# vinhisreal/YOLO-LitePi

Hardware: AMD Instinct MI355X
Metric: images/sec end-to-end (det+NMS+clf) 640x640 batch64 (higher is better)
Workload: dtype f16; 1 GPU; configs[2]: full det+NMS+ROI+ShuffleNetV2 pipeline, fp16, batch=64/GPU, 640x640, inputs resident in HBM; classifier=ShuffleNetV2 x1.0, 91 classes, seeded random weights, 64x64 ROIs, min_area=50, max_det=300, steps_in_flight=3, distinct_input_batches=4, global_batch=64, boxes_pre_area_filter_rank0=413

## Files before the change

yolo-litepi_amd/csrc/cls_net.h:

```cpp
#pragma once
#include "cls_fused.h"
#include "common.h"

namespace lp {

struct FusedS2W {
  const float* dw1;
  const float* dw1b;
  const u32x4_t* pwb1;
  const float* pwb1b;
  const u32x4_t* pw1;
  const float* pw1b;
  const float* dw2;
  const float* dw2b;
  const u32x4_t* pw2;
  const float* pw2b;
};

struct ClsFrontArgs {
  const uint8_t* rgb;
  const int* m_dyn;
  void* out;
  const u32x4_t* stem_w;
  const float* stem_b;
  FusedS2W s20;
  FusedBlockW s2[3];
  FusedS2W s30;
};

struct ClsBackArgs {
  const void* in;
  const int* m_dyn;
  FusedBlockW s3[7];
  FusedS2W s40;
  FusedBlockW s4[3];
  const u32x4_t* w5;
  const float* b5;
  const u32x4_t* wfc;
  const float* bfc;
  float* probs;
  int* ids;
  float* logits;
  lp_det* dets;
  const int* roi_img;
  const int* roi_slot;
  int max_det, nc, nc_p, logits_pitch;
};

void launch_cls_front(const ClsFrontArgs& a, int max_items, hipStream_t st);
void launch_cls_back(const ClsBackArgs& a, int max_items, hipStream_t st);
void pack_cls_stem(const std::vector<float>& w_oihw, const std::vector<float>& bias, std::vector<uint16_t>& frags, std::vector<float>& bias_cases);

}
```

yolo-litepi_amd/csrc/cls_net.hip:

```cpp
#include "cls_net.h"

namespace lp {

typedef _Float16 half_t;
typedef _Float16 half8 __attribute__((ext_vector_type(8)));
typedef _Float16 half4 __attribute__((ext_vector_type(4)));
typedef _Float16 half2v __attribute__((ext_vector_type(2)));
typedef float floatx4 __attribute__((ext_vector_type(4)));
typedef uint32_t u32x4 __attribute__((ext_vector_type(4)));

#define CN_THREADS 512
#define CN_WAVES 8

#define BF2 58
#define BFP2 64
#define BF3 116
#define BFP3 128
#define BF4 232
#define BFP4 240

template <int SMAX>
__device__ __forceinline__ void wload(u32x4 (&af)[SMAX], const u32x4_t* __restrict__ w, int t, int S, int lane) {
#pragma unroll
  for (int s = 0; s < SMAX; ++s) {
    af[s] = u32x4{0u, 0u, 0u, 0u};
    if (s < S) af[s] = w[((size_t)t * S + s) * 64 + lane];
  }
}

template <int SMAX, int PT>
__device__ __forceinline__ void gemm_acc(const u32x4 (&af)[SMAX], int S, int s0, const char* bsrc, int brow, int Kp, int p0, int lane,
                                         floatx4 (&acc)[PT]) {
  const int g = lane >> 4, col = lane & 15;
#pragma unroll
  for (int s = 0; s < SMAX; ++s) {
    if (s < S) {
      const half8 a = __builtin_bit_cast(half8, af[s]);
      const int kg = 4 * (s0 + s) + g;
#pragma unroll
      for (int p = 0; p < PT; ++p) {
        u32x4 v = u32x4{0u, 0u, 0u, 0u};
        if (kg * 8 < Kp) v = *reinterpret_cast<const u32x4*>(bsrc + (p0 + p * 16 + col) * brow + kg * 16);
        acc[p] = __builtin_amdgcn_mfma_f32_16x16x32_f16(a, __builtin_bit_cast(half8, v), acc[p], 0, 0, 0);
      }
    }
  }
}

template <int PT> __device__ __forceinline__ void zero_acc(floatx4 (&acc)[PT]) {
#pragma unroll
  for (int p = 0; p < PT; ++p) acc[p] = floatx4{0.f, 0.f, 0.f, 0.f};
}

template <int PT>
__device__ __forceinline__ void store_relu(char* dst, int drow, int p0, int t, const float* __restrict__ bias, const floatx4 (&acc)[PT],
                                           int lane) {
  const int g = lane >> 4, col = lane & 15;
  const int ch0 = t * 16 + 4 * g;
  const floatx4 b = *reinterpret_cast<const floatx4*>(bias + ch0);
#pragma unroll
  for (int p = 0; p < PT; ++p) {
    half4 q;
#pragma unroll
    for (int i = 0; i < 4; ++i) q[i] = (half_t)fmaxf(acc[p][i] + b[i], 0.f);
    *reinterpret_cast<half4*>(dst + (p0 + p * 16 + col) * drow + ch0 * 2) = q;
  }
}

template <int C, int WIN, int WOUT, int STRIDE>
__device__ __forceinline__ void dwconv(const char* in, int irow, char* out, int orow, const float* __restrict__ w,
                                       const float* __restrict__ b, int nroi, int tid) {
  constexpr int CG = C / 8;
  const int items = nroi * WOUT * WOUT * CG;
  for (int i = tid; i < items; i += CN_THREADS) {
    const int cg = i % CG, px = i / CG;
    const int r = px / (WOUT * WOUT), pp = px - r * (WOUT * WOUT);
    const int oy = pp / WOUT, ox = pp - oy * WOUT;
    float acc[8];
    {
      const floatx4 b0 = *reinterpret_cast<const floatx4*>(b + cg * 8), b1 = *reinterpret_cast<const floatx4*>(b + cg * 8 + 4);
#pragma unroll
      for (int j = 0; j < 4; ++j) { acc[j] = b0[j]; acc[4 + j] = b1[j]; }
    }
#pragma unroll 1
    for (int ky = 0; ky < 3; ++ky) {
      const int iy = oy * STRIDE - 1 + ky;
      if (iy < 0 || iy >= WIN) continue;
      const char* rowp = in + ((r * WIN + iy) * WIN) * irow + cg * 16;
      const float* wrow = w + (ky * 3) * C + cg * 8;
#pragma unroll
      for (int kx = 0; kx < 3; ++kx) {
        const int ix = ox * STRIDE - 1 + kx;
        const bool ok = ix >= 0 && ix < WIN;
        u32x4 raw = u32x4{0u, 0u, 0u, 0u};
        if (ok) raw = *reinterpret_cast<const u32x4*>(rowp + ix * irow);
        const half8 v = __builtin_bit_cast(half8, raw);
        const floatx4 w0 = *reinterpret_cast<const floatx4*>(wrow + kx * C);
        const floatx4 w1 = *reinterpret_cast<const floatx4*>(wrow + kx * C + 4);
#pragma unroll
        for (int j = 0; j < 4; ++j) {
          acc[j] = fmaf((float)v[j], w0[j], acc[j]);
          acc[4 + j] = fmaf((float)v[4 + j], w1[j], acc[4 + j]);
        }
      }
    }
    half8 o;
#pragma unroll
    for (int j = 0; j < 8; ++j) o[j] = (half_t)acc[j];
    *reinterpret_cast<half8*>(out + px * orow + cg * 16) = o;
  }
}

__device__ __forceinline__ int shuffle_phys(int l, int bf, int bfp) { return l < bf ? l : bfp + (l - bf); }

template <int BFP, int NB>
__device__ __forceinline__ void stage_biases(float* BI, const FusedBlockW* blk, int tid) {
  constexpr int Q = BFP / 4;
  for (int i = tid; i < NB * 2 * Q; i += CN_THREADS) {
    const int b = i / (2 * Q), rem = i - b * 2 * Q, which = rem / Q, j = rem - which * Q;
    const float* src = which ? blk[b].b2 : blk[b].b1;
    *reinterpret_cast<floatx4*>(BI + (size_t)(b * 2 + which) * BFP + 4 * j) = *reinterpret_cast<const floatx4*>(src + 4 * j);
  }
}

template <int C>
__device__ __forceinline__ void stage_dw(float* dst, const float* __restrict__ w, const float* __restrict__ b, int tid) {
  constexpr int Q = 10 * C / 4;
  for (int i = tid; i < Q; i += CN_THREADS)
    *reinterpret_cast<floatx4*>(dst + 4 * i) = i < 9 * C / 4 ? *reinterpret_cast<const floatx4*>(w + 4 * i) : *reinterpret_cast<const floatx4*>(b + 4 * (i - 9 * C / 4));
}

template <int BF, int BFP, int W, int PT, int ROUNDS, bool PREF = true>
__device__ __forceinline__ void s1_block(char* X, int xrow, char* T1, char* T2, int trow, const FusedBlockW& bw, const u32x4_t* w1n, int nroi,
                                         int p0, int tile0, int tstride, u32x4 (&f1)[ROUNDS][BFP / 32 + ((BFP % 32) ? 1 : 0)], int tid, float* DW, const float* BI) {
  constexpr int TT = BFP / 16, S = BFP / 32 + ((BFP % 32) ? 1 : 0);
  const int lane = tid & 63;
  const int g = lane >> 4, col = lane & 15;
  constexpr int NDW4 = 10 * BFP / 4, DWPT = (NDW4 + CN_THREADS - 1) / CN_THREADS;
  floatx4 dwreg[DWPT];
#pragma unroll
  for (int k = 0; k < DWPT; ++k) {
    int idx = tid + k * CN_THREADS;
    idx = idx < NDW4 ? idx : NDW4 - 1;
    dwreg[k] = idx < 9 * BFP / 4 ? *reinterpret_cast<const floatx4*>(bw.dw + 4 * idx) : *reinterpret_cast<const floatx4*>(bw.dwb + 4 * (idx - 9 * BFP / 4));
  }
  u32x4 f2[ROUNDS][S];
  floatx4 acc[ROUNDS][PT];
  int tc[ROUNDS];
  bool live[ROUNDS];
#pragma unroll
  for (int r = 0; r < ROUNDS; ++r) {
    const int t = tile0 + r * tstride;
    live[r] = t < TT;
    tc[r] = live[r] ? t : TT - 1;
  }
  if (PREF) {
#pragma unroll
    for (int r = 0; r < ROUNDS; ++r) wload<S>(f2[r], bw.w2, tc[r], S, lane);
  } else {
#pragma unroll
    for (int r = 0; r < ROUNDS; ++r) wload<S>(f1[r], bw.w1, tc[r], S, lane);
  }
#pragma unroll
  for (int r = 0; r < ROUNDS; ++r) {
    zero_acc<PT>(acc[r]);
    gemm_acc<S, PT>(f1[r], S, 0, X + BFP * 2, xrow, BFP, p0, lane, acc[r]);
    if (live[r]) store_relu<PT>(T1, trow, p0, tc[r], BI, acc[r], lane);
  }
  asm volatile("" ::: "memory");
  if (PREF) {
    if (w1n) {
#pragma unroll
      for (int r = 0; r < ROUNDS; ++r) wload<S>(f1[r], w1n, tc[r], S, lane);
    }
  } else {
#pragma unroll
    for (int r = 0; r < ROUNDS; ++r) wload<S>(f2[r], bw.w2, tc[r], S, lane);
  }
#pragma unroll
  for (int k = 0; k < DWPT; ++k) {
    const int idx = tid + k * CN_THREADS;
    if (idx < NDW4) *reinterpret_cast<floatx4*>(DW + 4 * idx) = dwreg[k];
  }
  __syncthreads();
  dwconv<BFP, W, W, 1>(T1, trow, T2, trow, DW, DW + 9 * BFP, nroi, tid);
  __syncthreads();
  half4 x1v[ROUNDS][PT];
#pragma unroll
  for (int r = 0; r < ROUNDS; ++r) {
    zero_acc<PT>(acc[r]);
    gemm_acc<S, PT>(f2[r], S, 0, T2, trow, BFP, p0, lane, acc[r]);
#pragma unroll
    for (int p = 0; p < PT; ++p) x1v[r][p] = *reinterpret_cast<const half4*>(X + (p0 + p * 16 + col) * xrow + (tc[r] * 16 + 4 * g) * 2);
  }
  __syncthreads();
#pragma unroll
  for (int r = 0; r < ROUNDS; ++r) {
    if (live[r]) {
      const int ch0 = tc[r] * 16 + 4 * g;
      const floatx4 bias = *reinterpret_cast<const floatx4*>(BI + BFP + ch0);
#pragma unroll
      for (int p = 0; p < PT; ++p) {
#pragma unroll
        for (int i = 0; i < 4; ++i) {
          const int c = ch0 + i;
          if (c < BF) {
            half2v pr;
            pr[0] = x1v[r][p][i];
            pr[1] = (half_t)fmaxf(acc[r][p][i] + bias[i], 0.f);
            *reinterpret_cast<half2v*>(X + (p0 + p * 16 + col) * xrow + shuffle_phys(2 * c, BF, BFP) * 2) = pr;
          }
        }
      }
    }
  }
  __syncthreads();
}

#define CF_IN 16
#define CF_RA 12352
#define CF_POOL (CF_RA + 49152)
#define CF_X2 (CF_POOL + 16384)
#define CF_LDS (CF_X2 + 17408)
#define CF_DW (10 * 64 * 4)
#define CF_BI (3 * 2 * 64 * 4)
#define CF_S2 ((10 * 24 + 10 * 64 + 10 * 128 + 10 * 128) * 4)
#define CF_POOLROW 64
#define CF_T1ROW 144
#define CF_X2ROW 272
#define CF_X3ROW 528

__global__ __launch_bounds__(CN_THREADS) void cls_front_kernel(const ClsFrontArgs a) {
  extern __shared__ __attribute__((aligned(16))) char smem[];
  const int tid0 = threadIdx.x, lane0 = tid0 & 63;
  const int R = *a.m_dyn;
  if ((int)blockIdx.x >= R) return;
  char* IN = smem + CF_IN;
  char* RA = smem + CF_RA;
  char* POOL = smem + CF_POOL;
  char* X2 = smem + CF_X2;
  char* T2 = smem;
  for (int i = tid0; i < 64 * CF_X2ROW / 16; i += CN_THREADS) *reinterpret_cast<u32x4*>(X2 + i * 16) = u32x4{0u, 0u, 0u, 0u};
  if (tid0 < 2) *reinterpret_cast<u32x4*>(smem + (tid0 ? CF_IN + 12288 : 0)) = u32x4{0u, 0u, 0u, 0u};
  stage_biases<BFP2, 3>(reinterpret_cast<float*>(smem + CF_LDS + CF_DW), a.s2, tid0);
  float* S2P = reinterpret_cast<float*>(smem + CF_LDS + CF_DW + CF_BI);
  stage_dw<24>(S2P, a.s20.dw1, a.s20.dw1b, tid0);
  stage_dw<64>(S2P + 240, a.s20.dw2, a.s20.dw2b, tid0);
  stage_dw<128>(S2P + 240 + 640, a.s30.dw1, a.s30.dw1b, tid0);
  stage_dw<128>(S2P + 240 + 640 + 1280, a.s30.dw2, a.s30.dw2b, tid0);
  const half8 sa0 = __builtin_bit_cast(half8, a.stem_w[lane0]), sa1 = __builtin_bit_cast(half8, a.stem_w[64 + lane0]);

  for (int r = blockIdx.x; r < R; r += gridDim.x) {
    int tid = tid0, lane = lane0;
    asm volatile("" : "+v"(tid), "+v"(lane));
    const int wave = __builtin_amdgcn_readfirstlane(tid >> 6);
    const int g = lane >> 4, col = lane & 15;
    {
      const u32x4* src = reinterpret_cast<const u32x4*>(a.rgb + (size_t)r * 12288);
      for (int i = tid; i < 768; i += CN_THREADS) *reinterpret_cast<u32x4*>(IN + i * 16) = src[i];
    }
    u32x4 fpw1[1];
    wload<1>(fpw1, a.s20.pw1, wave & 3, 1, lane);
    __syncthreads();

    for (int pt = wave * 8; pt < wave * 8 + 8; ++pt) {
      const int oy = pt >> 1, ox = (pt & 1) * 16 + col;
      const int b0 = 6 * ox - 3;
      uint32_t w0 = 0u, w1 = 0u;
      if (g < 3) {
        const int iy = 2 * oy - 1 + g;
        const int sh = b0 & 3, al = b0 - sh;
        const char* rowp = IN + (iy < 0 ? 0 : iy) * 192 + al;
        const uint32_t d0 = *reinterpret_cast<const uint32_t*>(rowp), d1 = *reinterpret_cast<const uint32_t*>(rowp + 4),
                       d2 = *reinterpret_cast<const uint32_t*>(rowp + 8);
        w0 = __builtin_amdgcn_alignbyte(d1, d0, sh);
        w1 = __builtin_amdgcn_alignbyte(d2, d1, sh);
        if (ox == 0) w0 &= 0xFF000000u;
        if (iy < 0) { w0 = 0u; w1 = 0u; }
      } else {
#pragma unroll
        for (int ky = 0; ky < 3; ++ky) {
          const int iy = 2 * oy - 1 + ky;
          const uint32_t v = iy < 0 ? 0u : (uint32_t) * reinterpret_cast<const uint8_t*>(IN + iy * 192 + b0 + 8);
          w0 |= v << (8 * ky);
        }
      }
      typedef uint32_t u32x4l __attribute__((ext_vector_type(4)));
      u32x4l hb;
      hb[0] = __builtin_amdgcn_perm(0x64646464u, w0, 0x04010400u);
      hb[1] = __builtin_amdgcn_perm(0x64646464u, w0, 0x04030402u);
      hb[2] = __builtin_amdgcn_perm(0x64646464u, w1, 0x04010400u);
      hb[3] = __builtin_amdgcn_perm(0x64646464u, w1, 0x04030402u);
      half8 bf = __builtin_bit_cast(half8, hb);
#pragma unroll
      for (int j = 0; j < 8; ++j) bf[j] = bf[j] - (half_t)1024.f;
      floatx4 c0 = floatx4{0.f, 0.f, 0.f, 0.f}, c1 = floatx4{0.f, 0.f, 0.f, 0.f};
      c0 = __builtin_amdgcn_mfma_f32_16x16x32_f16(sa0, bf, c0, 0, 0, 0);
      c1 = __builtin_amdgcn_mfma_f32_16x16x32_f16(sa1, bf, c1, 0, 0, 0);
      const int ci = (oy == 0 ? 1 : 0) | (ox == 0 ? 2 : 0);
      const floatx4 bb0 = *reinterpret_cast<const floatx4*>(a.stem_b + ci * 32 + 4 * g);
      char* o = RA + (oy * 32 + ox) * 48;
      half4 q;
#pragma unroll
      for (int i = 0; i < 4; ++i) q[i] = (half_t)fmaxf(c0[i] + bb0[i], 0.f);
      *reinterpret_cast<half4*>(o + 8 * g) = q;
      if (g < 2) {
        const floatx4 bb1 = *reinterpret_cast<const floatx4*>(a.stem_b + ci * 32 + 16 + 4 * g);
#pragma unroll
        for (int i = 0; i < 4; ++i) q[i] = (half_t)fmaxf(c1[i] + bb1[i], 0.f);
        *reinterpret_cast<half4*>(o + 32 + 8 * g) = q;
      }
    }
    __syncthreads();
    for (int i = tid; i < 768; i += CN_THREADS) {
      const int cg = i % 3, px = i / 3;
      const int oy = px >> 4, ox = px & 15;
      half8 m;
#pragma unroll
      for (int j = 0; j < 8; ++j) m[j] = (half_t)-65504.f;
#pragma unroll
      for (int ky = 0; ky < 3; ++ky) {
#pragma unroll
        for (int kx = 0; kx < 3; ++kx) {
          const int iy = 2 * oy - 1 + ky, ix = 2 * ox - 1 + kx;
          if (iy >= 0 && ix >= 0) {
            const half8 v = *reinterpret_cast<const half8*>(RA + (iy * 32 + ix) * 48 + cg * 16);
#pragma unroll
            for (int j = 0; j < 8; ++j) m[j] = v[j] > m[j] ? v[j] : m[j];
          }
        }
      }
      *reinterpret_cast<half8*>(POOL + px * CF_POOLROW + cg * 16) = m;
    }
    __syncthreads();

    char* T1 = RA;
    char* D1 = RA + 256 * CF_T1ROW;
    u32x4 fy[2];
    {
      const int t = wave & 3, p0 = (wave >> 2) * 128;
      floatx4 acc[8];
      zero_acc<8>(acc);
      gemm_acc<1, 8>(fpw1, 1, 0, POOL, CF_POOLROW, 24, p0, lane, acc);
      store_relu<8>(T1, CF_T1ROW, p0, t, a.s20.pw1b, acc, lane);
      if (wave < 4) wload<2>(fy, a.s20.pwb1, t, 1, lane); else wload<2>(fy, a.s20.pw2, t, 2, lane);
      dwconv<24, 16, 8, 2>(POOL, CF_POOLROW, D1, 64, S2P, S2P + 9 * 24, 1, tid);
    }
    __syncthreads();
    dwconv<64, 16, 8, 2>(T1, CF_T1ROW, T2, CF_T1ROW, S2P + 240, S2P + 240 + 9 * 64, 1, tid);
    __syncthreads();
    u32x4 f1[1][2];
    {
      const int t = wave & 3, which = wave >> 2;
      floatx4 acc[4];
      zero_acc<4>(acc);
      if (which == 0) gemm_acc<2, 4>(fy, 1, 0, D1, 64, 24, 0, lane, acc);
      else gemm_acc<2, 4>(fy, 2, 0, T2, CF_T1ROW, 64, 0, lane, acc);
      wload<2>(f1[0], a.s2[0].w1, t, 2, lane);
      const float* bias = which == 0 ? a.s20.pwb1b : a.s20.pw2b;
      const int ch0 = t * 16 + 4 * g;
      const floatx4 b = *reinterpret_cast<const floatx4*>(bias + ch0);
#pragma unroll
      for (int p = 0; p < 4; ++p) {
#pragma unroll
        for (int i = 0; i < 4; ++i) {
          const int c = ch0 + i;
          if (c < BF2)
            *reinterpret_cast<half_t*>(X2 + (p * 16 + col) * CF_X2ROW + shuffle_phys(2 * c + which, BF2, BFP2) * 2) =
                (half_t)fmaxf(acc[p][i] + b[i], 0.f);
        }
      }
    }
    __syncthreads();
#pragma unroll 1
    for (int b = 0; b < 3; ++b)
      s1_block<BF2, BFP2, 8, 2, 1>(X2, CF_X2ROW, RA, T2, CF_T1ROW, a.s2[b], b + 1 < 3 ? a.s2[b + 1].w1 : nullptr, 1, (wave >> 2) * 32, wave & 3,
                                   4, f1, tid, reinterpret_cast<float*>(smem + CF_LDS), reinterpret_cast<const float*>(smem + CF_LDS + CF_DW) + b * 2 * BFP2);

    char* T1c = RA;
    char* D1c = RA + 64 * CF_X2ROW;
    char* T2c = D1c + 16 * CF_X2ROW;
    char* X3 = T2c + 16 * CF_X2ROW;
    {
      u32x4 fa[4], fb[4], fc[4];
      wload<4>(fa, a.s30.pw1, wave, 4, lane);
      wload<4>(fb, a.s30.pwb1, wave, 4, lane);
      wload<4>(fc, a.s30.pw2, wave, 4, lane);
      for (int i = tid; i < 16 * CF_X3ROW / 16; i += CN_THREADS) *reinterpret_cast<u32x4*>(X3 + i * 16) = u32x4{0u, 0u, 0u, 0u};
      floatx4 acc[4];
      zero_acc<4>(acc);
      gemm_acc<4, 4>(fa, 4, 0, X2, CF_X2ROW, 128, 0, lane, acc);
      store_relu<4>(T1c, CF_X2ROW, 0, wave, a.s30.pw1b, acc, lane);
      dwconv<128, 8, 4, 2>(X2, CF_X2ROW, D1c, CF_X2ROW, S2P + 880, S2P + 880 + 9 * 128, 1, tid);
      __syncthreads();
      dwconv<128, 8, 4, 2>(T1c, CF_X2ROW, T2c, CF_X2ROW, S2P + 2160, S2P + 2160 + 9 * 128, 1, tid);
      __syncthreads();
      floatx4 y1[1], y2[1];
      zero_acc<1>(y1);
      zero_acc<1>(y2);
      gemm_acc<4, 1>(fb, 4, 0, D1c, CF_X2ROW, 128, 0, lane, y1);
      gemm_acc<4, 1>(fc, 4, 0, T2c, CF_X2ROW, 128, 0, lane, y2);
      const int ch0 = wave * 16 + 4 * g;
      const floatx4 b1 = *reinterpret_cast<const floatx4*>(a.s30.pwb1b + ch0), b2 = *reinterpret_cast<const floatx4*>(a.s30.pw2b + ch0);
#pragma unroll
      for (int i = 0; i < 4; ++i) {
        const int c = ch0 + i;
        if (c < BF3) {
          half2v pr;
          pr[0] = (half_t)fmaxf(y1[0][i] + b1[i], 0.f);
          pr[1] = (half_t)fmaxf(y2[0][i] + b2[i], 0.f);
          *reinterpret_cast<half2v*>(X3 + col * CF_X3ROW + shuffle_phys(2 * c, BF3, BFP3) * 2) = pr;
        }
      }
    }
    __syncthreads();
    {
      const int px = tid >> 5, ck = tid & 31;
      *reinterpret_cast<u32x4*>(reinterpret_cast<char*>(a.out) + ((size_t)r * 16 + px) * 512 + ck * 16) =
          *reinterpret_cast<const u32x4*>(X3 + px * CF_X3ROW + ck * 16);
    }
    __syncthreads();
  }
}

#define CB_RB 33792
#define CB_RC (CB_RB + 31744)
#define CB_X4 (CB_RC + 17408)
#define CB_LDS (CB_X4 + 15616)
#define CB_DW (10 * 240 * 4)
#define CB_BI3 (7 * 2 * 128 * 4)
#define CB_BI (CB_BI3 + 3 * 2 * 240 * 4)
#define CB_S2 ((10 * 256 + 10 * 240) * 4)
#define CB_T3ROW 272
#define CB_T4ROW 496
#define CB_X4ROW 976
#define CB_MROW 2064

__global__ __launch_bounds__(CN_THREADS) void cls_back_kernel(const ClsBackArgs a) {
  extern __shared__ __attribute__((aligned(16))) char smem[];
  const int tid0 = threadIdx.x, lane0 = tid0 & 63;
  const int R = *a.m_dyn;
  const int ngroups = (R + 3) >> 2;
  if ((int)blockIdx.x >= ngroups) return;
  char* X3 = smem;
  char* RB = smem + CB_RB;
  char* RC = smem + CB_RC;
  char* X4 = smem + CB_X4;
  for (int i = tid0; i < 16 * CB_X4ROW / 16; i += CN_THREADS) *reinterpret_cast<u32x4*>(X4 + i * 16) = u32x4{0u, 0u, 0u, 0u};
  stage_biases<BFP3, 7>(reinterpret_cast<float*>(smem + CB_LDS + CB_DW), a.s3, tid0);
  stage_biases<BFP4, 3>(reinterpret_cast<float*>(smem + CB_LDS + CB_DW + CB_BI3), a.s4, tid0);
  float* S2P = reinterpret_cast<float*>(smem + CB_LDS + CB_DW + CB_BI);
  stage_dw<256>(S2P, a.s40.dw1, a.s40.dw1b, tid0);
  stage_dw<240>(S2P + 2560, a.s40.dw2, a.s40.dw2b, tid0);

  for (int grp = blockIdx.x; grp < ngroups; grp += gridDim.x) {
    int tid = tid0, lane = lane0;
    asm volatile("" : "+v"(tid), "+v"(lane));
    const int wave = __builtin_amdgcn_readfirstlane(tid >> 6);
    const int g = lane >> 4, col = lane & 15;
    const int roi0 = grp * 4;
    const int nroi = (R - roi0) < 4 ? (R - roi0) : 4;
    u32x4 f3[1][4];
    wload<4>(f3[0], a.s3[0].w1, wave, 4, lane);
    for (int i = tid; i < 64 * 32; i += CN_THREADS) {
      const int px = i >> 5, ck = i & 31;
      u32x4 v = u32x4{0u, 0u, 0u, 0u};
      if (px < nroi * 16) v = *reinterpret_cast<const u32x4*>(reinterpret_cast<const char*>(a.in) + ((size_t)roi0 * 16 + px) * 512 + ck * 16);
      *reinterpret_cast<u32x4*>(X3 + px * CF_X3ROW + ck * 16) = v;
    }
    __syncthreads();
#pragma unroll 1
    for (int b = 0; b < 7; ++b)
      s1_block<BF3, BFP3, 4, 4, 1>(X3, CF_X3ROW, RB, RC, CB_T3ROW, a.s3[b], b + 1 < 7 ? a.s3[b + 1].w1 : nullptr, 4, 0, wave, 8, f3, tid,
                                   reinterpret_cast<float*>(smem + CB_LDS), reinterpret_cast<const float*>(smem + CB_LDS + CB_DW) + b * 2 * BFP3);

    char* T1 = RB;
    char* D1 = RC;
    char* T2 = RC + 16 * CF_X3ROW;
    u32x4 f4[2][8];
    {
      const int t0 = wave, t1 = wave + 8 < 15 ? wave + 8 : 14;
      const bool live1 = wave + 8 < 15;
      floatx4 y1[2][1];
      {
        u32x4 fb[2][8];
        wload<8>(fb[0], a.s40.pwb1, t0, 8, lane);
        wload<8>(fb[1], a.s40.pwb1, t1, 8, lane);
        dwconv<256, 4, 2, 2>(X3, CF_X3ROW, D1, CF_X3ROW, S2P, S2P + 9 * 256, 4, tid);
        __syncthreads();
        zero_acc<1>(y1[0]);
        zero_acc<1>(y1[1]);
        gemm_acc<8, 1>(fb[0], 8, 0, D1, CF_X3ROW, 256, 0, lane, y1[0]);
        gemm_acc<8, 1>(fb[1], 8, 0, D1, CF_X3ROW, 256, 0, lane, y1[1]);
      }
      asm volatile("" ::: "memory");
      {
        u32x4 fa[2][8];
        wload<8>(fa[0], a.s40.pw1, t0, 8, lane);
        wload<8>(fa[1], a.s40.pw1, t1, 8, lane);
        floatx4 acc[4];
        zero_acc<4>(acc);
        gemm_acc<8, 4>(fa[0], 8, 0, X3, CF_X3ROW, 256, 0, lane, acc);
        store_relu<4>(T1, CB_T4ROW, 0, t0, a.s40.pw1b, acc, lane);
        zero_acc<4>(acc);
        gemm_acc<8, 4>(fa[1], 8, 0, X3, CF_X3ROW, 256, 0, lane, acc);
        if (live1) store_relu<4>(T1, CB_T4ROW, 0, t1, a.s40.pw1b, acc, lane);
      }
      u32x4 fc[2][8];
      wload<8>(fc[0], a.s40.pw2, t0, 8, lane);
      wload<8>(fc[1], a.s40.pw2, t1, 8, lane);
      __syncthreads();
      dwconv<240, 4, 2, 2>(T1, CB_T4ROW, T2, CB_T4ROW, S2P + 2560, S2P + 2560 + 9 * 240, 4, tid);
      __syncthreads();
#pragma unroll
      for (int r = 0; r < 2; ++r) {
        const int t = r ? t1 : t0;
        floatx4 y2[1];
        zero_acc<1>(y2);
        gemm_acc<8, 1>(fc[r], 8, 0, T2, CB_T4ROW, 240, 0, lane, y2);
        if (r == 0 || live1) {
          const int ch0 = t * 16 + 4 * g;
          const floatx4 b1 = *reinterpret_cast<const floatx4*>(a.s40.pwb1b + ch0), b2 = *reinterpret_cast<const floatx4*>(a.s40.pw2b + ch0);
#pragma unroll
          for (int i = 0; i < 4; ++i) {
            const int c = ch0 + i;
            if (c < BF4) {
              half2v pr;
              pr[0] = (half_t)fmaxf(y1[r][0][i] + b1[i], 0.f);
              pr[1] = (half_t)fmaxf(y2[0][i] + b2[i], 0.f);
              *reinterpret_cast<half2v*>(X4 + col * CB_X4ROW + shuffle_phys(2 * c, BF4, BFP4) * 2) = pr;
            }
          }
        }
      }
      asm volatile("" ::: "memory");
      wload<8>(f4[0], a.s4[0].w1, t0, 8, lane);
      wload<8>(f4[1], a.s4[0].w1, t1, 8, lane);
    }
    __syncthreads();
#pragma unroll 1
    for (int b = 0; b < 3; ++b)
      s1_block<BF4, BFP4, 2, 1, 2, true>(X4, CB_X4ROW, RB, RB + 16 * CB_T4ROW, CB_T4ROW, a.s4[b], b + 1 < 3 ? a.s4[b + 1].w1 : nullptr, 4, 0, wave, 8, f4, tid,
                                         reinterpret_cast<float*>(smem + CB_LDS), reinterpret_cast<const float*>(smem + CB_LDS + CB_DW + CB_BI3) + b * 2 * BFP4);

    char* Mn = RC;
    float* LG = reinterpret_cast<float*>(RC + 4 * CB_MROW);
    {
      u32x4 fa[8], fb[8];
      wload<8>(fa, a.w5 + (size_t)(wave * 8) * 15 * 64, 0, 8, lane);
#pragma unroll 1
      for (int tq = 0; tq < 8; ++tq) {
        const int t = wave * 8 + tq;
        const u32x4_t* wt = a.w5 + (size_t)t * 15 * 64;
#pragma unroll
        for (int s = 0; s < 8; ++s) fb[s] = s < 7 ? wt[(8 + s) * 64 + lane] : u32x4{0u, 0u, 0u, 0u};
        floatx4 acc[1];
        zero_acc<1>(acc);
        gemm_acc<8, 1>(fa, 8, 0, X4, CB_X4ROW, 480, 0, lane, acc);
        if (tq + 1 < 8) wload<8>(fa, a.w5 + (size_t)(t + 1) * 15 * 64, 0, 8, lane);
        gemm_acc<8, 1>(fb, 7, 8, X4, CB_X4ROW, 480, 0, lane, acc);
        const int ch0 = t * 16 + 4 * g;
        const floatx4 bias = *reinterpret_cast<const floatx4*>(a.b5 + ch0);
        half4 q;
#pragma unroll
        for (int i = 0; i < 4; ++i) {
          float v = fmaxf(acc[0][i] + bias[i], 0.f);
          v += __shfl_xor(v, 1);
          v += __shfl_xor(v, 2);
          q[i] = (half_t)(v * 0.25f);
        }
        if ((col & 3) == 0) *reinterpret_cast<half4*>(Mn + (col >> 2) * CB_MROW + ch0 * 2) = q;
      }
    }
    __syncthreads();
    {
      const int Tfc = a.nc_p >> 4;
      for (int t = wave; t < Tfc; t += CN_WAVES) {
        floatx4 acc = floatx4{0.f, 0.f, 0.f, 0.f};
#pragma unroll 1
        for (int s0 = 0; s0 < 32; s0 += 8) {
          u32x4 af[8];
#pragma unroll
          for (int u = 0; u < 8; ++u) af[u] = a.wfc[((size_t)t * 32 + s0 + u) * 64 + lane];
#pragma unroll
          for (int u = 0; u < 8; ++u) {
            u32x4 v = u32x4{0u, 0u, 0u, 0u};
            if (col < 4) v = *reinterpret_cast<const u32x4*>(Mn + col * CB_MROW + (4 * (s0 + u) + g) * 16);
            acc = __builtin_amdgcn_mfma_f32_16x16x32_f16(__builtin_bit_cast(half8, af[u]), __builtin_bit_cast(half8, v), acc, 0, 0, 0);
          }
        }
        const int c0 = t * 16 + 4 * g;
        if (col < 4) {
#pragma unroll
          for (int i = 0; i < 4; ++i) LG[col * a.nc_p + c0 + i] = acc[i] + a.bfc[c0 + i];
        }
      }
    }
    __syncthreads();
    if (wave < nroi) {
      const int r = roi0 + wave;
      const float* l = LG + wave * a.nc_p;
      float mx = -INFINITY;
      for (int c = lane; c < a.nc; c += 64) mx = fmaxf(mx, l[c]);
      for (int o = 32; o > 0; o >>= 1) mx = fmaxf(mx, __shfl_xor(mx, o));
      float sum = 0.f;
      for (int c = lane; c < a.nc; c += 64) sum += expf(l[c] - mx);
      for (int o = 32; o > 0; o >>= 1) sum += __shfl_xor(sum, o);
      float best = -1.f;
      int best_c = 0x7fffffff;
      for (int c = lane; c < a.nc; c += 64) {
        const float pr = expf(l[c] - mx) / sum;
        if (a.probs) a.probs[(long)r * a.nc + c] = pr;
        if (pr > best) { best = pr; best_c = c; }
      }
      for (int o = 32; o > 0; o >>= 1) {
        const float ob = __shfl_xor(best, o);
        const int oc = __shfl_xor(best_c, o);
        if (ob > best || (ob == best && oc < best_c)) { best = ob; best_c = oc; }
      }
      if (lane == 0) {
        if (a.ids) a.ids[r] = best_c;
        if (a.dets) {
          lp_det* d = a.dets + (long)a.roi_img[r] * a.max_det + a.roi_slot[r];
          d->cls_class = best_c;
          d->cls_conf = best;
        }
      }
      if (a.logits)
        for (int c = lane; c < a.nc; c += 64) a.logits[(long)r * a.logits_pitch + c] = l[c];
    }
    __syncthreads();
  }
}

void launch_cls_front(const ClsFrontArgs& a, int max_items, hipStream_t st) {
  set_max_dynamic_lds(reinterpret_cast<const void*>(cls_front_kernel), 160 * 1024);
  int grid = max_items < 512 ? max_items : 512;
  if (grid < 1) grid = 1;
  LP_LAUNCH(cls_front_kernel, dim3(grid), dim3(CN_THREADS), CF_LDS + CF_DW + CF_BI + CF_S2, st, a);
  LP_HIP(hipGetLastError());
}

void launch_cls_back(const ClsBackArgs& a, int max_items, hipStream_t st) {
  LP_CHECK(a.nc_p % 16 == 0 && a.nc_p <= 1024 && (size_t)4 * CB_MROW + (size_t)4 * a.nc_p * 4 <= 17408, LP_ERR_STATE,
           "fused classifier: %d classes do not fit the logits buffer", a.nc);
  set_max_dynamic_lds(reinterpret_cast<const void*>(cls_back_kernel), 160 * 1024);
  int grid = (max_items + 3) / 4;
  if (grid > 256) grid = 256;
  if (grid < 1) grid = 1;
  LP_LAUNCH(cls_back_kernel, dim3(grid), dim3(CN_THREADS), CB_LDS + CB_DW + CB_BI + CB_S2, st, a);
  LP_HIP(hipGetLastError());
}

void pack_cls_stem(const std::vector<float>& w, const std::vector<float>& bias, std::vector<uint16_t>& frags, std::vector<float>& bias_cases) {
  const double scale = 1.0 / 255.0 / 0.34, shift = 0.18 / 0.34;
  frags.assign((size_t)2 * 64 * 8, 0);
  for (int t = 0; t < 2; ++t)
    for (int lane = 0; lane < 64; ++lane) {
      const int gq = lane >> 4, m = lane & 15, co = t * 16 + m;
      if (co >= 24) continue;
      for (int j = 0; j < 8; ++j) {
        int ky, kb;
        if (gq < 3) { ky = gq; kb = j; }
        else if (j < 3) { ky = j; kb = 8; }
        else continue;
        const int kx = kb / 3, c = kb % 3;
        frags[((size_t)t * 64 + lane) * 8 + j] = f32_to_f16((float)((double)w[(((size_t)co * 3 + c) * 3 + ky) * 3 + kx] * scale));
      }
    }
  bias_cases.assign((size_t)4 * 32, 0.f);
  for (int ci = 0; ci < 4; ++ci)
    for (int co = 0; co < 24; ++co) {
      double s = 0.0;
      for (int ky = 0; ky < 3; ++ky)
        for (int kx = 0; kx < 3; ++kx) {
          if ((ci & 1) && ky == 0) continue;
          if ((ci & 2) && kx == 0) continue;
          for (int c = 0; c < 3; ++c) s += (double)w[(((size_t)co * 3 + c) * 3 + ky) * 3 + kx];
        }
      bias_cases[(size_t)ci * 32 + co] = (float)((double)bias[co] - shift * s);
    }
}

}
```

Before: 121,300 images/sec.

## Shrink classifier front LDS footprint to fit two workgroups per CU

Reworks the classifier front kernel's LDS plan so its total shared-memory use fits in half of the 160 KiB, allowing two 512-thread workgroups per CU. The pool buffer now aliases the start of LDS at a tighter 48-byte row pitch, X3 aliases LDS start, and stage-3.0 depthwise parameters are prefetched into registers mid-kernel and written into the dead RA region instead of being staged up front. The full X2 zeroing is replaced by zeroing only the padding columns each iteration. It also adds optional env-gated per-block clock stamps for profiling; these are off by default but add a null-pointer check in both kernels.

```diff
diff --git a/yolo-litepi_amd/csrc/cls_net.h b/yolo-litepi_amd/csrc/cls_net.h
--- a/yolo-litepi_amd/csrc/cls_net.h
+++ b/yolo-litepi_amd/csrc/cls_net.h
@@ -26,6 +26,7 @@
   FusedS2W s20;
   FusedBlockW s2[3];
   FusedS2W s30;
+  unsigned long long* stamps;
 };
 
 struct ClsBackArgs {
@@ -45,6 +46,7 @@
   const int* roi_img;
   const int* roi_slot;
   int max_det, nc, nc_p, logits_pitch;
+  unsigned long long* stamps;
 };
 
 void launch_cls_front(const ClsFrontArgs& a, int max_items, hipStream_t st);
diff --git a/yolo-litepi_amd/csrc/cls_net.hip b/yolo-litepi_amd/csrc/cls_net.hip
--- a/yolo-litepi_amd/csrc/cls_net.hip
+++ b/yolo-litepi_amd/csrc/cls_net.hip
@@ -18,6 +18,10 @@
 #define BFP3 128
 #define BF4 232
 #define BFP4 240
+
+#define CN_STAMP(k)                                 \
+  if (a.stamps && first_pass && threadIdx.x == 0)   \
+    a.stamps[(size_t)blockIdx.x * 16 + (k)] = ((k) == 0 || (k) == 15) ? wall_clock64() : clock64();
 
 template <int SMAX>
 __device__ __forceinline__ void wload(u32x4 (&af)[SMAX], const u32x4_t* __restrict__ w, int t, int S, int lane) {
@@ -219,38 +223,44 @@
 
 #define CF_IN 16
 #define CF_RA 12352
-#define CF_POOL (CF_RA + 49152)
-#define CF_X2 (CF_POOL + 16384)
+#define CF_X2 (CF_RA + 40960)
 #define CF_LDS (CF_X2 + 17408)
 #define CF_DW (10 * 64 * 4)
 #define CF_BI (3 * 2 * 64 * 4)
-#define CF_S2 ((10 * 24 + 10 * 64 + 10 * 128 + 10 * 128) * 4)
-#define CF_POOLROW 64
+#define CF_S2 ((10 * 24 + 10 * 64) * 4)
+#define CF_S30P (CF_RA + 26112)
+#define CF_TOTAL (CF_LDS + CF_DW + CF_BI + CF_S2)
+static_assert(CF_TOTAL <= 81920, "cls_front: two workgroups per CU need at most half of the 160 KiB each");
+static_assert(CF_S30P + 2 * 10 * 128 * 4 <= CF_X2, "cls_front: stage3.0's depthwise parameters must end inside RA");
+#define CF_POOLROW 48
 #define CF_T1ROW 144
 #define CF_X2ROW 272
 #define CF_X3ROW 528
 
-__global__ __launch_bounds__(CN_THREADS) void cls_front_kernel(const ClsFrontArgs a) {
+__global__ __launch_bounds__(CN_THREADS, 4) void cls_front_kernel(const ClsFrontArgs a) {
   extern __shared__ __attribute__((aligned(16))) char smem[];
   const int tid0 = threadIdx.x, lane0 = tid0 & 63;
   const int R = *a.m_dyn;
   if ((int)blockIdx.x >= R) return;
+  {
+    const bool first_pass = true;
+    CN_STAMP(0)
+    CN_STAMP(1)
+  }
   char* IN = smem + CF_IN;
   char* RA = smem + CF_RA;
-  char* POOL = smem + CF_POOL;
+  char* POOL = smem;
   char* X2 = smem + CF_X2;
   char* T2 = smem;
-  for (int i = tid0; i < 64 * CF_X2ROW / 16; i += CN_THREADS) *reinterpret_cast<u32x4*>(X2 + i * 16) = u32x4{0u, 0u, 0u, 0u};
-  if (tid0 < 2) *reinterpret_cast<u32x4*>(smem + (tid0 ? CF_IN + 12288 : 0)) = u32x4{0u, 0u, 0u, 0u};
   stage_biases<BFP2, 3>(reinterpret_cast<float*>(smem + CF_LDS + CF_DW), a.s2, tid0);
   float* S2P = reinterpret_cast<float*>(smem + CF_LDS + CF_DW + CF_BI);
   stage_dw<24>(S2P, a.s20.dw1, a.s20.dw1b, tid0);
   stage_dw<64>(S2P + 240, a.s20.dw2, a.s20.dw2b, tid0);
-  stage_dw<128>(S2P + 240 + 640, a.s30.dw1, a.s30.dw1b, tid0);
-  stage_dw<128>(S2P + 240 + 640 + 1280, a.s30.dw2, a.s30.dw2b, tid0);
+  const float* S30P = reinterpret_cast<const float*>(smem + CF_S30P);
   const half8 sa0 = __builtin_bit_cast(half8, a.stem_w[lane0]), sa1 = __builtin_bit_cast(half8, a.stem_w[64 + lane0]);
 
   for (int r = blockIdx.x; r < R; r += gridDim.x) {
+    const bool first_pass = r == (int)blockIdx.x;
     int tid = tid0, lane = lane0;
     asm volatile("" : "+v"(tid), "+v"(lane));
     const int wave = __builtin_amdgcn_readfirstlane(tid >> 6);
@@ -262,6 +272,7 @@
     u32x4 fpw1[1];
     wload<1>(fpw1, a.s20.pw1, wave & 3, 1, lane);
     __syncthreads();
+    CN_STAMP(2)
 
     for (int pt = wave * 8; pt < wave * 8 + 8; ++pt) {
       const int oy = pt >> 1, ox = (pt & 1) * 16 + col;
@@ -333,12 +344,14 @@
       *reinterpret_cast<half8*>(POOL + px * CF_POOLROW + cg * 16) = m;
     }
     __syncthreads();
+    CN_STAMP(3)
 
     char* T1 = RA;
     char* D1 = RA + 256 * CF_T1ROW;
     u32x4 fy[2];
     {
       const int t = wave & 3, p0 = (wave >> 2) * 128;
+      if (tid < 64 * 6) *reinterpret_cast<uint32_t*>(X2 + (tid / 6) * CF_X2ROW + ((tid % 6) < 3 ? BF2 * 2 : (BFP2 + BF2) * 2) + ((tid % 6) % 3) * 4) = 0u;
       floatx4 acc[8];
       zero_acc<8>(acc);
       gemm_acc<1, 8>(fpw1, 1, 0, POOL, CF_POOLROW, 24, p0, lane, acc);
@@ -352,6 +365,16 @@
     u32x4 f1[1][2];
     {
       const int t = wave & 3, which = wave >> 2;
+      floatx4 q30[2];
+#pragma unroll
+      for (int k = 0; k < 2; ++k) {
+        int idx = tid + k * CN_THREADS;
+        idx = idx < 640 ? idx : 639;
+        const int h = idx >= 320, j = idx - h * 320;
+        const float* w = h ? a.s30.dw2 : a.s30.dw1;
+        const float* bq = h ? a.s30.dw2b : a.s30.dw1b;
+        q30[k] = j < 288 ? *reinterpret_cast<const floatx4*>(w + 4 * j) : *reinterpret_cast<const floatx4*>(bq + 4 * (j - 288));
+      }
       floatx4 acc[4];
       zero_acc<4>(acc);
       if (which == 0) gemm_acc<2, 4>(fy, 1, 0, D1, 64, 24, 0, lane, acc);
@@ -370,17 +393,22 @@
                 (half_t)fmaxf(acc[p][i] + b[i], 0.f);
         }
       }
-    }
-    __syncthreads();
+#pragma unroll
+      for (int k = 0; k < 2; ++k)
+        if (tid + k * CN_THREADS < 640) *reinterpret_cast<floatx4*>(smem + CF_S30P + (tid + k * CN_THREADS) * 16) = q30[k];
+    }
+    __syncthreads();
+    CN_STAMP(4)
 #pragma unroll 1
     for (int b = 0; b < 3; ++b)
       s1_block<BF2, BFP2, 8, 2, 1>(X2, CF_X2ROW, RA, T2, CF_T1ROW, a.s2[b], b + 1 < 3 ? a.s2[b + 1].w1 : nullptr, 1, (wave >> 2) * 32, wave & 3,
                                    4, f1, tid, reinterpret_cast<float*>(smem + CF_LDS), reinterpret_cast<const float*>(smem + CF_LDS + CF_DW) + b * 2 * BFP2);
+    CN_STAMP(5)
 
     char* T1c = RA;
     char* D1c = RA + 64 * CF_X2ROW;
     char* T2c = D1c + 16 * CF_X2ROW;
-    char* X3 = T2c + 16 * CF_X2ROW;
+    char* X3 = smem;
     {
       u32x4 fa[4], fb[4], fc[4];
       wload<4>(fa, a.s30.pw1, wave, 4, lane);
@@ -391,9 +419,9 @@
       zero_acc<4>(acc);
       gemm_acc<4, 4>(fa, 4, 0, X2, CF_X2ROW, 128, 0, lane, acc);
       store_relu<4>(T1c, CF_X2ROW, 0, wave, a.s30.pw1b, acc, lane);
-      dwconv<128, 8, 4, 2>(X2, CF_X2ROW, D1c, CF_X2ROW, S2P + 880, S2P + 880 + 9 * 128, 1, tid);
+      dwconv<128, 8, 4, 2>(X2, CF_X2ROW, D1c, CF_X2ROW, S30P, S30P + 9 * 128, 1, tid);
       __syncthreads();
-      dwconv<128, 8, 4, 2>(T1c, CF_X2ROW, T2c, CF_X2ROW, S2P + 2160, S2P + 2160 + 9 * 128, 1, tid);
+      dwconv<128, 8, 4, 2>(T1c, CF_X2ROW, T2c, CF_X2ROW, S30P + 1280, S30P + 1280 + 9 * 128, 1, tid);
       __syncthreads();
       floatx4 y1[1], y2[1];
       zero_acc<1>(y1);
@@ -414,11 +442,14 @@
       }
     }
     __syncthreads();
+    CN_STAMP(6)
     {
       const int px = tid >> 5, ck = tid & 31;
       *reinterpret_cast<u32x4*>(reinterpret_cast<char*>(a.out) + ((size_t)r * 16 + px) * 512 + ck * 16) =
           *reinterpret_cast<const u32x4*>(X3 + px * CF_X3ROW + ck * 16);
     }
+    CN_STAMP(7)
+    CN_STAMP(15)
     __syncthreads();
   }
 }
@@ -442,6 +473,11 @@
   const int R = *a.m_dyn;
   const int ngroups = (R + 3) >> 2;
   if ((int)blockIdx.x >= ngroups) return;
+  {
+    const bool first_pass = true;
+    CN_STAMP(0)
+    CN_STAMP(1)
+  }
   char* X3 = smem;
   char* RB = smem + CB_RB;
   char* RC = smem + CB_RC;
@@ -454,6 +490,7 @@
   stage_dw<240>(S2P + 2560, a.s40.dw2, a.s40.dw2b, tid0);
 
   for (int grp = blockIdx.x; grp < ngroups; grp += gridDim.x) {
+    const bool first_pass = grp == (int)blockIdx.x;
     int tid = tid0, lane = lane0;
     asm volatile("" : "+v"(tid), "+v"(lane));
     const int wave = __builtin_amdgcn_readfirstlane(tid >> 6);
@@ -469,10 +506,12 @@
       *reinterpret_cast<u32x4*>(X3 + px * CF_X3ROW + ck * 16) = v;
     }
     __syncthreads();
+    CN_STAMP(2)
 #pragma unroll 1
     for (int b = 0; b < 7; ++b)
       s1_block<BF3, BFP3, 4, 4, 1>(X3, CF_X3ROW, RB, RC, CB_T3ROW, a.s3[b], b + 1 < 7 ? a.s3[b + 1].w1 : nullptr, 4, 0, wave, 8, f3, tid,
                                    reinterpret_cast<float*>(smem + CB_LDS), reinterpret_cast<const float*>(smem + CB_LDS + CB_DW) + b * 2 * BFP3);
+    CN_STAMP(3)
 
     char* T1 = RB;
     char* D1 = RC;
@@ -538,10 +577,12 @@
       wload<8>(f4[1], a.s4[0].w1, t1, 8, lane);
     }
     __syncthreads();
+    CN_STAMP(4)
 #pragma unroll 1
     for (int b = 0; b < 3; ++b)
       s1_block<BF4, BFP4, 2, 1, 2, true>(X4, CB_X4ROW, RB, RB + 16 * CB_T4ROW, CB_T4ROW, a.s4[b], b + 1 < 3 ? a.s4[b + 1].w1 : nullptr, 4, 0, wave, 8, f4, tid,
                                          reinterpret_cast<float*>(smem + CB_LDS), reinterpret_cast<const float*>(smem + CB_LDS + CB_DW + CB_BI3) + b * 2 * BFP4);
+    CN_STAMP(5)
 
     char* Mn = RC;
     float* LG = reinterpret_cast<float*>(RC + 4 * CB_MROW);
@@ -573,6 +614,7 @@
       }
     }
     __syncthreads();
+    CN_STAMP(6)
     {
       const int Tfc = a.nc_p >> 4;
       for (int t = wave; t < Tfc; t += CN_WAVES) {
@@ -597,6 +639,7 @@
       }
     }
     __syncthreads();
+    CN_STAMP(7)
     if (wave < nroi) {
       const int r = roi0 + wave;
       const float* l = LG + wave * a.nc_p;
@@ -629,27 +672,64 @@
       if (a.logits)
         for (int c = lane; c < a.nc; c += 64) a.logits[(long)r * a.logits_pitch + c] = l[c];
     }
-    __syncthreads();
-  }
-}
+    CN_STAMP(8)
+    CN_STAMP(15)
+    __syncthreads();
+  }
+}
+
+struct ClsStamps {
+  DevBuf buf;
+  int grid;
+  ClsStamps(int grid_, hipStream_t st) : grid(grid_) {
+    if (!path() || !*path()) return;
+    buf.alloc((size_t)grid * 16 * 8);
+    LP_HIP(hipMemsetAsync(buf.p, 0, (size_t)grid * 16 * 8, st));
+  }
+  static const char* path() {
+    static const char* p = getenv("LITEPI_CLS_STAMPS");
+    return p;
+  }
+  unsigned long long* dev() { return buf.p ? buf.as<unsigned long long>() : nullptr; }
+  void dump(unsigned long long tag, int max_items, hipStream_t st) {
+    if (!buf.p) return;
+    LP_HIP(hipStreamSynchronize(st));
+    std::vector<unsigned long long> hs((size_t)grid * 16);
+    LP_HIP(hipMemcpy(hs.data(), buf.p, hs.size() * 8, hipMemcpyDeviceToHost));
+    if (FILE* f = fopen(path(), "ab")) {
+      const unsigned long long hdr[4] = {tag, (unsigned long long)grid, (unsigned long long)max_items, 0ull};
+      fwrite(hdr, 8, 4, f);
+      fwrite(hs.data(), 8, hs.size(), f);
+      fclose(f);
+    }
+  }
+};
 
 void launch_cls_front(const ClsFrontArgs& a, int max_items, hipStream_t st) {
-  set_max_dynamic_lds(reinterpret_cast<const void*>(cls_front_kernel), 160 * 1024);
   int grid = max_items < 512 ? max_items : 512;
   if (grid < 1) grid = 1;
-  LP_LAUNCH(cls_front_kernel, dim3(grid), dim3(CN_THREADS), CF_LDS + CF_DW + CF_BI + CF_S2, st, a);
+  ClsFrontArgs k = a;
+  ClsStamps stamps(grid, st);
+  k.stamps = stamps.dev();
+  set_max_dynamic_lds(reinterpret_cast<const void*>(cls_front_kernel), 160 * 1024);
+  LP_LAUNCH(cls_front_kernel, dim3(grid), dim3(CN_THREADS), CF_TOTAL, st, k);
   LP_HIP(hipGetLastError());
+  stamps.dump(0x434c5346ull , max_items, st);
 }
 
 void launch_cls_back(const ClsBackArgs& a, int max_items, hipStream_t st) {
   LP_CHECK(a.nc_p % 16 == 0 && a.nc_p <= 1024 && (size_t)4 * CB_MROW + (size_t)4 * a.nc_p * 4 <= 17408, LP_ERR_STATE,
            "fused classifier: %d classes do not fit the logits buffer", a.nc);
-  set_max_dynamic_lds(reinterpret_cast<const void*>(cls_back_kernel), 160 * 1024);
   int grid = (max_items + 3) / 4;
   if (grid > 256) grid = 256;
   if (grid < 1) grid = 1;
-  LP_LAUNCH(cls_back_kernel, dim3(grid), dim3(CN_THREADS), CB_LDS + CB_DW + CB_BI + CB_S2, st, a);
+  ClsBackArgs k = a;
+  ClsStamps stamps(grid, st);
+  k.stamps = stamps.dev();
+  set_max_dynamic_lds(reinterpret_cast<const void*>(cls_back_kernel), 160 * 1024);
+  LP_LAUNCH(cls_back_kernel, dim3(grid), dim3(CN_THREADS), CB_LDS + CB_DW + CB_BI + CB_S2, st, k);
   LP_HIP(hipGetLastError());
+  stamps.dump(0x434c5342ull , max_items, st);
 }
 
 void pack_cls_stem(const std::vector<float>& w, const std::vector<float>& bias, std::vector<uint16_t>& frags, std::vector<float>& bias_cases) {
```

Result: faster. 123,600 images/sec, median of 6 (+1.9%).
